# Zeudon/sound-event-localization-detection

Hardware: AMD Instinct MI355X
Metric: training clips/sec (4ch FOA 60s@24kHz) (higher is better)
Workload: dtype bf16; 1 GPU; crnn FOA 4-ch 60s clips, bs=32 windows (BASELINE configs[1]); parallelism=dp1

## Files before the change

### include/seld_hip.h

```cpp
#ifndef SELD_HIP_H_
#define SELD_HIP_H_

#include <stdint.h>

#ifdef __cplusplus
extern "C" {
#endif

int seld_init(int device);
int seld_shutdown(void);
int seld_version(void);
const char* seld_last_error(void);

int seld_set_mel_filterbank(const float* fb_host);

int seld_set_window(const float* window_host);

int seld_default_tables(float* window960, float* fb481x64, int* mel_b0_64, float* mel_wd_24x64,
                        float* mel_wu_24x64);

int64_t seld_num_frames(int64_t L);

int seld_logmel_f32(const float* pcm, int64_t N, int64_t C, int64_t L, float* out, int layout, void* stream);
int seld_logmel_i16(const int16_t* pcm, int64_t N, int64_t C, int64_t L, float* out, int layout, void* stream);
// ... 114 lines not shown
                         seld_guard_record* guard, void* stream);

int seld_multi_adam_guarded(const void* const* grad, const int32_t* grad_is_bf16, float* const* param,
                            float* const* exp_avg, float* const* exp_avg_sq, void* const* low_bf16, const int64_t* lengths,
                            int count, const float* lr, const float* step, float beta1, float beta2, float eps,
                            float weight_decay, float grad_scale, float* const* ema, float ema_decay,
                            const seld_guard_record* guard, void* stream);

int seld_multi_cast(const void* const* src, void* const* dst, const int64_t* lengths, int count, int bf16_to_fp32,
                    void* stream);

int seld_layernorm_supported(int64_t D);
int64_t seld_layernorm_workspace_floats(int64_t rows, int64_t D);
int seld_layernorm_forward(const void* x, int is_bf16, int64_t rows, int64_t D, const float* weight, const float* bias,
                           float eps, int relu, void* y, float* mean_rstd, void* stream);
int seld_layernorm_backward(const void* x, const void* dy, int is_bf16, int64_t rows, int64_t D, const float* weight,
                            const float* bias, const float* mean_rstd, int relu, void* dx, float* dweight,
                            float* dbias, float* workspace, void* stream);

int seld_stream_delay(int64_t nanoseconds, void* stream);

int64_t seld_smr_loss_workspace_bytes(int64_t frames, int64_t cells_per_frame);
int seld_smr_loss(const void* logits, int logits_is_bf16, const uint16_t* mask, const float* dense_labels,
                  int64_t frames, int rows, int cols, int num_classes, float w_class, float w_aiur, float w_cl,
                  float* loss_out4, void* grad, void* workspace, void* stream);


int seld_gru_fold_bias(const float* b_ih, const float* b_hh, int64_t H, void* gi_bias, int out_is_bf16, float* b_hn,
                       void* stream);

int seld_gru_prepare(const float* b_ih, const float* b_hh, const void* w_hh, int w_is_bf16, int64_t H, void* gi_bias,
                     int out_is_bf16, float* b_hn, void* w_hh_t_bf16, void* stream);

int seld_gru_bias_grads(const float* partial, int64_t tiles, int64_t H, float* db_ih, float* db_hh, void* stream);

int seld_sum_chunks(const void* partial, int in_is_bf16, int64_t chunks, int64_t count, void* out, int out_is_bf16,
                    void* stream);

int seld_sum_chunks_columns(const void* partial, int in_is_bf16, int64_t chunks, int64_t rows, int64_t C, int64_t F,
                            void* out, int out_is_bf16, void* stream);

int64_t seld_column_sums_blocks(int64_t rows, int64_t n_cols);
int seld_column_sums(const void* g, int in_is_bf16, int64_t rows, int64_t n_cols, float* partial, void* out, int out_is_bf16,
                     void* stream);

int seld_multi_sum_chunks(const void* const* partial, void* const* out, const int64_t* counts, const int32_t* chunks,
                          const int32_t* flags, int count, void* stream);
int seld_multi_column_sums_scratch(const int64_t* rows, const int64_t* n_cols, int count, int64_t* partial_floats);
int seld_multi_column_sums(const void* const* g, void* const* out, const int64_t* rows, const int64_t* n_cols,
                           const int32_t* flags, int count, float* partial, int64_t partial_floats, void* stream);

int seld_gru_dwhh_finish(const void* p_gi, const void* p_n, int in_is_bf16, int64_t chunks, int64_t H, void* dw_hh,
                         int out_is_bf16, void* stream);

int seld_conv_weight_flip_transpose(const void* w, int elem_bytes, int64_t O, int64_t I, void* wt, void* stream);

int seld_conv3x3_wgrad_supported(int64_t F, int64_t Cin, int64_t Cout);
int64_t seld_conv3x3_wgrad_workspace_floats(int64_t B, int64_t T, int64_t F, int64_t Cin, int64_t Cout);
int seld_conv3x3_wgrad(const void* x, const void* dy, int64_t B, int64_t T, int64_t F, int64_t Cin, int64_t Cout,
                       void* dw, int dw_is_bf16, float* workspace, void* stream);

int seld_conv3x3_dgrad_supported(int64_t F, int64_t Cin, int64_t Cout);
int seld_conv3x3_dgrad(const void* dy, const void* w, int64_t B, int64_t T, int64_t F, int64_t Cin, int64_t Cout,
                       void* dx, void* stream);

int seld_convfirst_supported(int64_t F, int64_t Cin, int64_t Cout);
int64_t seld_convfirst_workspace_floats(int backward);
int seld_convfirst_forward(const void* in, const void* w, int w_is_bf16, int64_t w_sco, int64_t w_sci, int64_t w_sr,
                           int64_t w_ss, int64_t B, int64_t T, int64_t F, const float* bn_weight, const float* bn_bias,
                           float* running_mean, float* running_var, float momentum, float eps, void* y,
                           float* mean_invstd, float* scale_shift, float* workspace, int phases, void* stream);
int seld_convfirst_backward(const void* in, const void* w, int w_is_bf16, int64_t w_sco, int64_t w_sci, int64_t w_sr,
                            int64_t w_ss, const void* dy, int64_t B, int64_t T, int64_t F, const float* mean_invstd,
                            const float* scale_shift, void* dw, int dw_is_bf16, int64_t dw_sco, int64_t dw_sci,
                            int64_t dw_sr, int64_t dw_ss, float* dgamma, float* dbeta, float* workspace, int phases,
                            void* stream);

int64_t seld_conv_tail_workspace_floats(int C);
int seld_conv_tail_forward(const void* x, const void* residual, int is_bf16, int64_t rows, int C, int pool,
                           const float* weight, const float* bias, float* running_mean, float* running_var,
                           float momentum, float eps, int training, void* y, float* mean_invstd, float* scale_shift,
                           float* workspace, void* stream);
int seld_conv_tail_backward(const void* x, const void* residual, const void* dy, int is_bf16, int64_t rows, int C,
                            int pool, const float* mean_invstd, const float* scale_shift, void* dx, void* dresidual,
                            float* dweight, float* dbias, float* workspace, void* stream);

int seld_dwconv1d(const void* x, int is_bf16, const float* weight, const float* bias, int64_t B, int64_t T, int D, int K,
                  int flip_taps, void* y, void* stream);
int64_t seld_dwconv1d_wgrad_rows(int64_t B, int64_t T);
int seld_dwconv1d_wgrad(const void* x, const void* dy, int is_bf16, int64_t B, int64_t T, int D, int K, float* partial,
                        void* stream);

int64_t seld_gru_tile_rows(void);
int seld_gru_forward(const void* gi, int is_bf16, const void* w_hh_bf16, const float* b_hn, int64_t B,
                     int64_t T, int64_t H, void* y, void* saved_tile, void* stream);

int seld_gru_backward(const void* dy_tile, const void* saved_tile, const void* y, int is_bf16,
                      const void* w_hh_t_bf16, int64_t tiles, int64_t T, int64_t H, void* dg_tile, float* dbias,
                      void* stream);

int seld_gru_backward_direct(const void* dy, const void* saved_tile, const void* y, int is_bf16,
                             const void* w_hh_t_bf16, int64_t B, int64_t T, int64_t H, void* dgi, void* dghn,
                             float* dbias, void* stream);

int seld_gru_to_tile(const void* src, int elem_bytes, int64_t B, int64_t T, int ns, void* dst, void* stream);
int seld_gru_from_pair_tile(const void* dg_tile, int elem_bytes, int64_t B, int64_t T, void* dgi, void* dghn,
// ... 64 lines not shown
```

### sound-event-localization-detection_amd/csrc/conv3x3_image.h

```cpp
#pragma once

#include <hip/hip_runtime.h>

namespace seld {
namespace conv3x3 {

typedef __attribute__((ext_vector_type(8))) __bf16 bf16x8;
typedef __attribute__((ext_vector_type(4))) short s16x4;
typedef __attribute__((ext_vector_type(8))) short s16x8;
typedef __attribute__((ext_vector_type(4))) float f32x4;
typedef __attribute__((address_space(3))) s16x4 lds_s16x4;

constexpr int kThreads = 256;
constexpr int kChannels = 64;
constexpr int kPitch = 80;

template <int F, int P>
struct Image {
  static_assert(F == 8 || F == 16 || F == 32, "frequency bins: 8, 16 or 32");
  static_assert(P % F == 0, "a chunk is whole time rows");
  static constexpr int TC = P / F;
  static constexpr int kRows = (TC + 2) * (F + 2);
  static constexpr int kLoads = (kRows * 8 + kThreads - 1) / kThreads;
};

template <int F>
__device__ __forceinline__ int image_row(int pos) {
  return (pos / F + 1) * (F + 2) + pos % F + 1;
}

template <int F>
__device__ __forceinline__ constexpr int tap_shift(int tap) {
  return (tap / 3 - 1) * (F + 2) + (tap % 3 - 1);
}

template <int F, int P>
__device__ __forceinline__ uint4 image_piece(const unsigned short* __restrict__ src, long clip_row, int t0, int T,
                                             int C, int c0, int piece) {
  const int r = piece >> 3, ch = piece & 7;
  const int tr = r / (F + 2), f = r - tr * (F + 2) - 1, t = t0 - 1 + tr;
  uint4 v = make_uint4(0u, 0u, 0u, 0u);
  if (r < Image<F, P>::kRows && t >= 0 && t < T && f >= 0 && f < F)
    v = *reinterpret_cast<const uint4*>(src + ((clip_row + t) * F + f) * C + c0 + ch * 8);
  return v;
}

__device__ __forceinline__ s16x4 tr_read(const unsigned short* base, int offset_shorts) {
  return __builtin_amdgcn_ds_read_tr16_b64_v4i16((lds_s16x4*)(base + offset_shorts));
}

__device__ __forceinline__ bf16x8 join(s16x4 lo, s16x4 hi) {
  const s16x8 v = __builtin_shufflevector(lo, hi, 0, 1, 2, 3, 4, 5, 6, 7);
  return __builtin_bit_cast(bf16x8, v);
}

}
}
```

### sound-event-localization-detection_amd/csrc/convwgrad.hip

```cpp
#include <hip/hip_bf16.h>

#include "conv3x3_image.h"
#include "seld_common.h"

namespace seld {

namespace {

using namespace conv3x3;

constexpr int kWgThreads = 512;
constexpr int kWgTile = 64;
constexpr int kWgKc = 128;
constexpr int kWgPitch = kPitch;
constexpr int kWgSumThreads = 256;
constexpr int kWgSumRows = 8;

template <int F>
struct WgradGeom {
  using Img = Image<F, kWgKc>;
  static constexpr int TC = Img::TC;
  static constexpr int XR = Img::kRows;
  static constexpr int kDyLoads = kWgKc * 8 / kWgThreads;
  static constexpr int kXLoads = (XR * 8 + kWgThreads - 1) / kWgThreads;
// ... 140 lines not shown
    }
  part[row][col] = s;
  __syncthreads();
  if (row != 0 || i >= count) return;
#pragma unroll
  for (int r = 1; r < kWgSumRows; ++r) {
    const float4 v = part[r][col];
    s.x += v.x; s.y += v.y; s.z += v.z; s.w += v.w;
  }
  if (kBf16) {
    const unsigned lo = static_cast<unsigned>(__bfloat16_as_ushort(__float2bfloat16(s.x))) |
                        (static_cast<unsigned>(__bfloat16_as_ushort(__float2bfloat16(s.y))) << 16);
    const unsigned hi = static_cast<unsigned>(__bfloat16_as_ushort(__float2bfloat16(s.z))) |
                        (static_cast<unsigned>(__bfloat16_as_ushort(__float2bfloat16(s.w))) << 16);
    *reinterpret_cast<uint2*>(static_cast<unsigned short*>(dw) + i) = make_uint2(lo, hi);
  } else {
    *reinterpret_cast<float4*>(static_cast<float*>(dw) + i) = s;
  }
}

struct WgradPlan {
  int chunks_per_clip = 0, chunks = 0, per_slab = 0, slabs = 0;
};

int time_rows_per_chunk(int64_t F) { return static_cast<int>(kWgKc / F); }

bool wgrad_supported(int64_t F, int64_t Cin, int64_t Cout) {
  return (F == 8 || F == 16 || F == 32) && Cin > 0 && Cout > 0 && Cin % kWgTile == 0 &&
         Cout % kWgTile == 0;
}

WgradPlan wgrad_plan(int64_t B, int64_t T, int64_t F, int64_t Cin, int64_t Cout, int num_cus) {
  WgradPlan pl;
  const int tc = time_rows_per_chunk(F);
  pl.chunks_per_clip = static_cast<int>((T + tc - 1) / tc);
  pl.chunks = static_cast<int>(B) * pl.chunks_per_clip;
  const long tiles = (Cin / kWgTile) * (Cout / kWgTile);
  const long want = ((num_cus > 0 ? num_cus : 256) + tiles - 1) / tiles;
  const long slabs = want < 1 ? 1 : (want > pl.chunks ? pl.chunks : want);
  pl.per_slab = static_cast<int>((pl.chunks + slabs - 1) / slabs);
  pl.slabs = (pl.chunks + pl.per_slab - 1) / pl.per_slab;
  return pl;
}

template <int F>
void launch_wgrad(const unsigned short* x, const unsigned short* dy, int T, int Cin, int Cout, const WgradPlan& pl,
                  float* ws, hipStream_t stream) {
  const dim3 grid(static_cast<unsigned>(Cin / kWgTile), static_cast<unsigned>(Cout / kWgTile),
                  static_cast<unsigned>(pl.slabs));
  hipLaunchKernelGGL(conv3x3_wgrad_kernel<F>, grid, dim3(kWgThreads), 0, stream, x, dy, T, Cin, Cout,
                     pl.chunks_per_clip, pl.chunks, pl.per_slab, ws);
}

}

}

extern "C" {

int seld_conv3x3_wgrad_supported(int64_t F, int64_t Cin, int64_t Cout) {
  return seld::wgrad_supported(F, Cin, Cout) ? 1 : 0;
}

int64_t seld_conv3x3_wgrad_workspace_floats(int64_t B, int64_t T, int64_t F, int64_t Cin, int64_t Cout) {
  using namespace seld;
  const DeviceState* st = current_state();
  if (!st || B <= 0 || T <= 0 || !wgrad_supported(F, Cin, Cout)) return 0;
  return static_cast<int64_t>(wgrad_plan(B, T, F, Cin, Cout, st->num_cus).slabs) * Cout * 9 * Cin;
}

int seld_conv3x3_wgrad(const void* x, const void* dy, int64_t B, int64_t T, int64_t F, int64_t Cin, int64_t Cout,
                       void* dw, int dw_is_bf16, float* workspace, void* stream_) {
  using namespace seld;
  const DeviceState* st = current_state();
  if (!st) return kErrNotInitialised;
  if (!x || !dy || !dw || !workspace || B <= 0 || T <= 0)
    return fail(kErrInvalidArgument, "seld_conv3x3_wgrad: bad argument");
  if (!wgrad_supported(F, Cin, Cout))
    return fail(kErrUnsupported, "seld_conv3x3_wgrad: F in {8, 16, 32} and channel counts % 64 == 0 required");
  if (((reinterpret_cast<uintptr_t>(x) | reinterpret_cast<uintptr_t>(dy) | reinterpret_cast<uintptr_t>(dw) |
        reinterpret_cast<uintptr_t>(workspace)) & 15) != 0)
    return fail(kErrInvalidArgument, "seld_conv3x3_wgrad: 16-byte aligned tensors required");
  const WgradPlan pl = wgrad_plan(B, T, F, Cin, Cout, st->num_cus);
  hipStream_t stream = static_cast<hipStream_t>(stream_);
  const unsigned short* xs = static_cast<const unsigned short*>(x);
  const unsigned short* ds = static_cast<const unsigned short*>(dy);
  const int t = static_cast<int>(T), ci = static_cast<int>(Cin), co = static_cast<int>(Cout);
  switch (F) {
    case 8: launch_wgrad<8>(xs, ds, t, ci, co, pl, workspace, stream); break;
    case 16: launch_wgrad<16>(xs, ds, t, ci, co, pl, workspace, stream); break;
    default: launch_wgrad<32>(xs, ds, t, ci, co, pl, workspace, stream); break;
  }
  SELD_HIP_TRY(hipGetLastError());
  const long count = static_cast<long>(Cout) * 9 * Cin;
  const long cols = kWgSumThreads / kWgSumRows;
  const dim3 grid(static_cast<unsigned>((count / 4 + cols - 1) / cols));
  if (dw_is_bf16)
    hipLaunchKernelGGL(conv3x3_wgrad_sum_kernel<true>, grid, dim3(kWgSumThreads), 0, stream, workspace, pl.slabs,
                       count, dw);
  else
    hipLaunchKernelGGL(conv3x3_wgrad_sum_kernel<false>, grid, dim3(kWgSumThreads), 0, stream, workspace, pl.slabs,
                       count, dw);
  SELD_HIP_TRY(hipGetLastError());
  return kOk;
}

}
```

### sound-event-localization-detection_amd/seld_gru.py

```python
import torch
import torch.nn.functional as F

import seld_native
import seld_overlap
from seld_linear import chunk_count, tall_chunks, tall_product

HIDDEN = 256
direct_backward = True


def applicable(module, x):
    low = torch.is_autocast_enabled() or x.dtype in (torch.bfloat16, torch.float16)
    if not low and not getattr(module, "allow_fp32", False):
        return False
    return (module.hidden_size == HIDDEN and module.bidirectional and module.batch_first and module.bias
            and x.dim() == 3 and x.dtype in (torch.float32, torch.bfloat16, torch.float16) and module.proj_size == 0)


class _BiGRULayer(torch.autograd.Function):
    @staticmethod
    def forward(ctx, x, w_ih, b_ih, w_hh, b_hh, overlap=False, feature_cf=None):
        ctx.overlap = overlap
        ctx.feature_cf = feature_cf
        if feature_cf is not None:
            c, f = feature_cf
            w_ih = w_ih.view(w_ih.shape[0], c, f).transpose(1, 2).reshape(w_ih.shape[0], f * c)
        low = torch.is_autocast_enabled() or x.dtype == torch.bfloat16
        cdt = torch.bfloat16 if low else torch.float32
        with torch.autocast(device_type="cuda", enabled=False):
            xc = x.to(cdt)
            need = x.requires_grad or w_ih.requires_grad or w_hh.requires_grad
            w_hh_t = None
            if b_ih.dtype == torch.float32 and b_hh.dtype == torch.float32 and b_ih.is_contiguous() and b_hh.is_contiguous():
                if (direct_backward and need and w_hh.is_contiguous()
                        and w_hh.dtype in (torch.float32, torch.bfloat16)):
                    gi_bias, b_hn, w_hh_t = seld_native.gru_prepare(b_ih, b_hh.reshape(-1), w_hh, cdt)
                else:
                    gi_bias, b_hn = seld_native.gru_fold_bias(b_ih, b_hh.reshape(-1), cdt)
            else:
                fold = b_hh.clone()
                fold[:, 2 * HIDDEN:] = 0
                gi_bias, b_hn = (b_ih + fold.reshape(-1)).to(cdt), b_hh[:, 2 * HIDDEN:]
            gi = F.linear(xc, w_ih.to(cdt), gi_bias)
            b, t, _ = gi.shape
            y, saved = seld_native.gru_forward(gi.view(b, t, 2, 3 * HIDDEN), w_hh, b_hn, need)
        ctx.save_for_backward(xc, w_ih, w_hh, y, saved if saved is not None else torch.empty(0),
                              w_hh_t if w_hh_t is not None else torch.empty(0))
        ctx.cdt = cdt
        ctx.dtypes = (w_ih.dtype, b_ih.dtype, w_hh.dtype, b_hh.dtype)
        return y

    @staticmethod
    def backward(ctx, dy):
        xc, w_ih, w_hh, y, saved, w_hh_t = ctx.saved_tensors
        cdt = ctx.cdt
        b, t, _ = y.shape
        h = HIDDEN
        n = b * t
        with torch.autocast(device_type="cuda", enabled=False):
            dyc = dy.to(y.dtype)
            seld_overlap.launch_pending(dy.device)
            dgi, dghn, dbias = seld_native.gru_backward(dyc, saved, y, w_hh, raw_bias=True,
                                                        w_hh_t=w_hh_t if w_hh_t.numel() else None, direct=direct_backward)
            dgi2 = dgi.view(n, 6 * h)
            x2 = xc.reshape(n, -1)
            t_wih, t_bih, t_whh, t_bhh = ctx.dtypes

            dw_ih = torch.empty((6 * h, x2.shape[1]), dtype=t_wih, device=dy.device)
            dw_hh = torch.empty((2, 3 * h, h), dtype=t_whh, device=dy.device)
            db_ih = torch.empty(6 * h, dtype=t_bih, device=dy.device)
            db_hh = torch.empty(6 * h, dtype=t_bhh, device=dy.device)

            def weight_grads():
                fp32 = [db if db.dtype == torch.float32 else torch.empty(6 * h, dtype=torch.float32, device=dy.device)
                        for db in (db_ih, db_hh)]
                seld_native.gru_bias_grads(dbias, out=fp32)
                for db, full in zip((db_ih, db_hh), fp32):
                    if db is not full:
                        db.copy_(full)
                tall_product(dgi2, x2, out=dw_ih, columns_cf=ctx.feature_cf)
                hp = seld_native.gru_previous_state(y).view(n, 2 * h)
                chunks = chunk_count(n, 6 * h, 2 * h)
                p_gi = tall_chunks(dgi2, hp, chunks)
                p_n = tall_chunks(dghn.view(n, 2 * h), hp, chunks)
                seld_native.gru_dwhh_finish(p_gi, p_n, dw_hh)

            dx = (dgi2 @ w_ih.to(cdt)).view_as(xc)
            if ctx.overlap:
                seld_overlap.submit(dy.device, [dgi, dghn, y, xc, dbias, dw_ih, dw_hh, db_ih, db_hh], weight_grads)
            elif seld_overlap.conv_wgrad_side and seld_overlap.enabled and dy.is_cuda:
                seld_overlap.launch_now(dy.device, [dgi, dghn, y, xc, dbias, dw_ih, dw_hh, db_ih, db_hh], weight_grads,
                                        last_of_stage=True, outputs=[dw_ih, dw_hh, db_ih, db_hh])
            else:
                weight_grads()
        return dx.to(dy.dtype) if dx.dtype != dy.dtype and not torch.is_autocast_enabled() else dx, \
            dw_ih.view_as(dw_ih), db_ih.view_as(db_ih), dw_hh.view_as(dw_hh), db_hh.view(2, 3 * h), None, None


from seld_pack import adjacent as _adjacent, join as _join, pack as _pack


def pack_parameters(module):
    with torch.no_grad():
        for layer in range(module.num_layers):
            for kind in ("weight_ih", "bias_ih", "weight_hh", "bias_hh"):
                _pack((getattr(module, f"{kind}_l{layer}"), getattr(module, f"{kind}_l{layer}_reverse")))


def bigru_forward(module, x, feature_cf=None, overlap=False, need_hn=True):
    overlap = overlap and seld_overlap.active(x)
    params = []
    for layer in range(module.num_layers):
        p = lambda name: getattr(module, f"{name}_l{layer}")
        pr = lambda name: getattr(module, f"{name}_l{layer}_reverse")
        group = (_join(p("weight_ih"), pr("weight_ih")), _join(p("bias_ih"), pr("bias_ih")),
                 _join(p("weight_hh"), pr("weight_hh")), _join(p("bias_hh"), pr("bias_hh")))
        params.append(seld_overlap.defer(*group) if overlap and layer > 0 else group)
    out = x
    finals = []
    for layer in range(module.num_layers):
        w_ih, b_ih, w_hh, b_hh = params[layer]
        out = _BiGRULayer.apply(out, w_ih, b_ih, w_hh.view(2, 3 * HIDDEN, HIDDEN), b_hh.view(2, 3 * HIDDEN),
                                overlap and layer > 0, feature_cf if layer == 0 else None)
        if need_hn:
            finals += [out[:, -1, :HIDDEN], out[:, 0, HIDDEN:]]
        if module.training and module.dropout > 0 and layer + 1 < module.num_layers:
            out = F.dropout(out, p=module.dropout, training=True)
    return out, (torch.stack(finals, dim=0) if need_hn else None)
```

### sound-event-localization-detection_amd/seld_native.py

```python
from __future__ import annotations

import ctypes
import os
import threading
from pathlib import Path

import torch

from seld_augment import PARAM_INTS as AUGMENT_PARAM_INTS, PATTERNS as AUGMENT_PATTERNS, check_channel_order

_HERE = Path(__file__).resolve().parent
LIB_PATH = Path(os.environ["SELD_HIP_LIB"]).resolve() if os.environ.get("SELD_HIP_LIB") else _HERE / "libseld_hip.so"

N_FFT = 960
HOP = 480
N_BINS = 481
N_MELS = 64

_lock = threading.Lock()
_lib = None
_initialised_devices = set()

_i64 = ctypes.c_int64
_int = ctypes.c_int
# ... 22 lines not shown
    for name in ("seld_stft_f32", "seld_stft_i16"):
        getattr(lib, name).argtypes = [_ptr, _i64, _i64, _i64, _ptr, _ptr]
    lib.seld_foa_intensity.argtypes = [_ptr, _i64, _i64, _ptr, _i64, _i64, _i64, _i64, _ptr]
    for fn in (lib.seld_logmel_iv_f32, lib.seld_logmel_iv_i16):
        fn.argtypes = [_ptr, _i64, _i64, _ptr, _i64, _i64, _i64, _i64, _ptr]
    for fn in (lib.seld_logmel_spectrum_f32, lib.seld_logmel_spectrum_i16):
        fn.argtypes = [_ptr, _i64, _i64, _i64, _ptr, _i64, _i64, _i64, _i64, _ptr, _ptr]
        fn.restype = ctypes.c_int
    for fn in (lib.seld_logmel_phasors_f32, lib.seld_logmel_phasors_i16):
        fn.argtypes = [_ptr, _i64, _i64, _i64, _ptr, _i64, _i64, _i64, _i64, _ptr, _ptr]
    lib.seld_phasor_pitch.restype = ctypes.c_int64
    lib.seld_gcc_phat_q15.argtypes = [_ptr, _i64, _i64, _i64, _ptr, _i64, _i64, _i64, _i64, _ptr]
    lib.seld_gcc_table_host.argtypes = [_ptr]
    lib.seld_gcc_phat.argtypes = [_ptr, _i64, _i64, _i64, _ptr, _i64, _i64, _i64, _i64, _ptr]
    lib.seld_labels_rasterise.argtypes = [_ptr, _i64, _i64, _int, _int, _ptr, _ptr]
    lib.seld_labels_expand.argtypes = [_ptr, _i64, _int, _ptr, _ptr]
    lib.seld_labels_rasterise_box.argtypes = [_ptr, _ptr, _i64, _i64, _int, _int, ctypes.c_double, ctypes.c_double, _ptr,
                                              _ptr]
    lib.seld_window_gather.argtypes = [_ptr, _i64, _i64, _ptr, _i64, _i64, _ptr, _ptr]
    lib.seld_window_gather_augment.argtypes = [_ptr, _i64, _int, _int, _ptr, _ptr, _i64, _i64, _ptr, ctypes.c_float, _ptr, _ptr]
    lib.seld_window_permute_mask.argtypes = [_ptr, _i64, _int, _int, _ptr, _ptr, _i64, _i64, _ptr, _ptr]
    lib.seld_foa_rotation_terms.argtypes = [_ptr, _i64, _i64, _int, _int, _ptr, _i64, _i64, _i64, _i64, _ptr]
    lib.seld_window_gather_rotate.argtypes = [_ptr, _ptr, _i64, _int, _int, _int, _int, _int, _int, _ptr, _ptr, _i64, _i64, _ptr,
                                              ctypes.c_float, _ptr, _ptr]
    lib.seld_window_permute_mask_rotate.argtypes = [_ptr, _i64, _int, _int, _ptr, _ptr, _i64, _i64, _ptr, _ptr]
    lib.seld_feature_moments_workspace.restype = _i64
    lib.seld_feature_moments_workspace.argtypes = [_i64, _int]
    lib.seld_feature_moments.argtypes = [_ptr, _i64, _int, _ptr, _ptr, _i64, _ptr]
    lib.seld_window_gather_affine.argtypes = [_ptr, _i64, _int, _ptr, _i64, _i64, _ptr, _ptr, _ptr, _ptr]
    lib.seld_window_gather_augment_affine.argtypes = [_ptr, _i64, _int, _int, _ptr, _ptr, _i64, _i64, _ptr, ctypes.c_float,
                                                      _ptr, _ptr, _ptr, _ptr]
    lib.seld_window_gather_rotate_affine.argtypes = [_ptr, _ptr, _i64, _int, _int, _int, _int, _int, _int, _ptr, _ptr, _i64,
                                                     _i64, _ptr, ctypes.c_float, _ptr, _ptr, _ptr, _ptr]
    lib.seld_softmax_mse_workspace_bytes.restype = _i64
    lib.seld_softmax_mse_workspace_bytes.argtypes = []
    lib.seld_softmax_mse.argtypes = [_ptr, _int, _ptr, _ptr, _i64, _int, ctypes.c_float, _ptr, _ptr, _ptr, _ptr]
    lib.seld_softmax_ce_workspace_bytes.restype = _i64
    lib.seld_softmax_ce_workspace_bytes.argtypes = []
    lib.seld_softmax_ce.argtypes = [_ptr, _int, _ptr, _ptr, _i64, _int, _ptr, ctypes.c_float, ctypes.c_float, _ptr, _ptr,
                                    _ptr, _ptr]
    lib.seld_scale_by_device_scalar.argtypes = [_ptr, _int, _i64, _ptr, _ptr]
    lib.seld_smr_loss_workspace_bytes.restype = _i64
    lib.seld_smr_loss_workspace_bytes.argtypes = [_i64, _i64]
    lib.seld_smr_loss.argtypes = [_ptr, _int, _ptr, _ptr, _i64, _int, _int, _int, ctypes.c_float, ctypes.c_float,
                                  ctypes.c_float, _ptr, _ptr, _ptr, _ptr]
    lib.seld_multi_cast.argtypes = [_ptr, _ptr, _ptr, _int, _int, _ptr]
    lib.seld_stream_delay.argtypes = [_i64, _ptr]
    lib.seld_gru_fold_bias.argtypes = [_ptr, _ptr, _i64, _ptr, _int, _ptr, _ptr]
    lib.seld_gru_prepare.argtypes = [_ptr, _ptr, _ptr, _int, _i64, _ptr, _int, _ptr, _ptr, _ptr]
    lib.seld_gru_bias_grads.argtypes = [_ptr, _i64, _i64, _ptr, _ptr, _ptr]
    lib.seld_sum_chunks.argtypes = [_ptr, _int, _i64, _i64, _ptr, _int, _ptr]
    lib.seld_sum_chunks_columns.argtypes = [_ptr, _int, _i64, _i64, _i64, _i64, _ptr, _int, _ptr]
    lib.seld_gru_dwhh_finish.argtypes = [_ptr, _ptr, _int, _i64, _i64, _ptr, _int, _ptr]
    lib.seld_column_sums.argtypes = [_ptr, _int, _i64, _i64, _ptr, _ptr, _int, _ptr]
    _pp, _pi64, _pi32 = ctypes.POINTER(ctypes.c_void_p), ctypes.POINTER(ctypes.c_int64), ctypes.POINTER(ctypes.c_int32)
    _f = ctypes.c_float
    lib.seld_multi_adam.argtypes = [_pp, _pi32, _pp, _pp, _pp, _pp, _pi64, _int, _ptr, _ptr, _f, _f, _f, _f, _f, _ptr]
    lib.seld_multi_grad_norm_scratch.argtypes = [_pi64, _int, _pi64]
    lib.seld_multi_grad_norm.argtypes = [_pp, _pi32, _pi64, _int, _f, _f, _int, _ptr, _i64, _ptr, _ptr]
    lib.seld_multi_adam_guarded.argtypes = [_pp, _pi32, _pp, _pp, _pp, _pp, _pi64, _int, _ptr, _ptr, _f, _f, _f, _f, _f, _pp, _f,
                                            _ptr, _ptr]
    lib.seld_multi_sum_chunks.argtypes = [_pp, _pp, _pi64, _pi32, _pi32, _int, _ptr]
    lib.seld_multi_column_sums_scratch.argtypes = [_pi64, _pi64, _int, _pi64]
    lib.seld_multi_column_sums.argtypes = [_pp, _pp, _pi64, _pi64, _pi32, _int, _ptr, _i64, _ptr]
    lib.seld_column_sums_blocks.argtypes = [_i64, _i64]
    lib.seld_column_sums_blocks.restype = ctypes.c_int64
    lib.seld_conv_weight_flip_transpose.argtypes = [_ptr, _int, _i64, _i64, _ptr, _ptr]
    lib.seld_conv3x3_wgrad_supported.argtypes = [_i64, _i64, _i64]
    lib.seld_conv3x3_wgrad_workspace_floats.restype = _i64
    lib.seld_conv3x3_wgrad_workspace_floats.argtypes = [_i64, _i64, _i64, _i64, _i64]
    lib.seld_conv3x3_wgrad.argtypes = [_ptr, _ptr, _i64, _i64, _i64, _i64, _i64, _ptr, _int, _ptr, _ptr]
    lib.seld_conv3x3_dgrad_supported.argtypes = [_i64, _i64, _i64]
    lib.seld_conv3x3_dgrad.argtypes = [_ptr, _ptr, _i64, _i64, _i64, _i64, _i64, _ptr, _ptr]
    lib.seld_convfirst_supported.argtypes = [_i64, _i64, _i64]
    lib.seld_convfirst_workspace_floats.restype = _i64
    lib.seld_convfirst_workspace_floats.argtypes = [_int]
    lib.seld_convfirst_forward.argtypes = [_ptr, _ptr, _int, _i64, _i64, _i64, _i64, _i64, _i64, _i64, _ptr, _ptr, _ptr, _ptr,
                                           ctypes.c_float, ctypes.c_float, _ptr, _ptr, _ptr, _ptr, _int, _ptr]
    lib.seld_convfirst_backward.argtypes = [_ptr, _ptr, _int, _i64, _i64, _i64, _i64, _ptr, _i64, _i64, _i64, _ptr, _ptr,
                                            _ptr, _int, _i64, _i64, _i64, _i64, _ptr, _ptr, _ptr, _int, _ptr]
    lib.seld_layernorm_supported.argtypes = [_i64]
    lib.seld_layernorm_workspace_floats.restype = _i64
    lib.seld_layernorm_workspace_floats.argtypes = [_i64, _i64]
    lib.seld_layernorm_forward.argtypes = [_ptr, _int, _i64, _i64, _ptr, _ptr, ctypes.c_float, _int, _ptr, _ptr, _ptr]
    lib.seld_layernorm_backward.argtypes = [_ptr, _ptr, _int, _i64, _i64, _ptr, _ptr, _ptr, _int, _ptr, _ptr, _ptr,
                                            _ptr, _ptr]
    lib.seld_conv_tail_workspace_floats.restype = _i64
    lib.seld_conv_tail_workspace_floats.argtypes = [_int]
    lib.seld_conv_tail_forward.argtypes = [_ptr, _ptr, _int, _i64, _int, _int, _ptr, _ptr, _ptr, _ptr, ctypes.c_float,
                                           ctypes.c_float, _int, _ptr, _ptr, _ptr, _ptr, _ptr]
    lib.seld_conv_tail_backward.argtypes = [_ptr, _ptr, _ptr, _int, _i64, _int, _int, _ptr, _ptr, _ptr, _ptr, _ptr, _ptr,
                                            _ptr, _ptr]
    lib.seld_dwconv1d.argtypes = [_ptr, _int, _ptr, _ptr, _i64, _i64, _int, _int, _int, _ptr, _ptr]
    lib.seld_dwconv1d_wgrad.argtypes = [_ptr, _ptr, _int, _i64, _i64, _int, _int, _ptr, _ptr]
    lib.seld_dwconv1d_wgrad_rows.argtypes = [_i64, _i64]
    lib.seld_dwconv1d_wgrad_rows.restype = ctypes.c_int64
    lib.seld_gru_to_tile.argtypes = [_ptr, _int, _i64, _i64, _int, _ptr, _ptr]
    lib.seld_gru_from_pair_tile.argtypes = [_ptr, _int, _i64, _i64, _ptr, _ptr, _ptr]
    lib.seld_gru_previous_state.argtypes = [_ptr, _int, _i64, _i64, _ptr, _ptr]
    lib.seld_gru_tile_rows.restype = _i64
    lib.seld_gru_tile_rows.argtypes = []
    lib.seld_gru_forward.argtypes = [_ptr, _int, _ptr, _ptr, _i64, _i64, _i64, _ptr, _ptr, _ptr]
    lib.seld_gru_backward.argtypes = [_ptr, _ptr, _ptr, _int, _ptr, _i64, _i64, _i64, _ptr, _ptr, _ptr]
    lib.seld_gru_backward_direct.argtypes = [_ptr, _ptr, _ptr, _int, _ptr, _i64, _i64, _i64, _ptr, _ptr, _ptr, _ptr]
    lib.seld_grid_decode.argtypes = [_ptr, _int, _i64, _i64, _i64, _i64, _ptr, _ptr, _i64, _i64, ctypes.c_float, _int,
                                     _ptr, _ptr, _ptr, _ptr, _ptr]
# ... 1197 lines not shown
    with _device_guard(ensure_init(device)):
        check(load_library().seld_multi_sum_chunks(src, dst, counts, chunks, flags, n, _stream_ptr(device)),
              "seld_multi_sum_chunks")


_column_scratch = {}
_retired_scratch = []


def multi_column_sums(pairs) -> None:
    pairs = list(pairs)
    if not pairs:
        return
    for g, out in pairs:
        if not column_sums_supported(g, out):
            raise SeldNativeError("multi_column_sums: g [rows, N] contiguous bf16 / fp32 with N % 8 == 0, out [N] contiguous")
    lib = load_library()
    n = len(pairs)
    src = (ctypes.c_void_p * n)(*[g.data_ptr() for g, _ in pairs])
    dst = (ctypes.c_void_p * n)(*[o.data_ptr() for _, o in pairs])
    rows = (ctypes.c_int64 * n)(*[g.shape[0] for g, _ in pairs])
    cols = (ctypes.c_int64 * n)(*[g.shape[1] for g, _ in pairs])
    flags = (ctypes.c_int32 * n)(*[_is_bf16(g) | (_is_bf16(o) << 1) for g, o in pairs])
    need_f = ctypes.c_int64(0)
    check(lib.seld_multi_column_sums_scratch(rows, cols, n, ctypes.byref(need_f)), "seld_multi_column_sums_scratch")
    device = pairs[0][0].device
    index = ensure_init(device)
    scratch = _column_scratch.get(index)
    if scratch is None or scratch.numel() < need_f.value:
        if torch.cuda.is_current_stream_capturing():
            raise SeldNativeError("multi_column_sums: the scratch must be sized by an eager call before a graph capture")
        if scratch is not None:
            _retired_scratch.append(scratch)
        scratch = torch.empty(max(need_f.value, 1 << 20), dtype=torch.float32, device=device)
        _column_scratch[index] = scratch
    with _device_guard(index):
        check(lib.seld_multi_column_sums(src, dst, rows, cols, flags, n, _p(scratch), scratch.numel(), _stream_ptr(device)),
              "seld_multi_column_sums")


def gru_dwhh_finish(p_gi: torch.Tensor, p_n: torch.Tensor, out: torch.Tensor) -> torch.Tensor:
    chunks = p_gi.shape[0]
    h = out.shape[2]
    if not (p_gi.is_contiguous() and p_n.is_contiguous() and out.is_contiguous() and p_gi.dtype == p_n.dtype
            and tuple(p_gi.shape) == (chunks, 6 * h, 2 * h) and tuple(p_n.shape) == (chunks, 2 * h, 2 * h)
            and tuple(out.shape) == (2, 3 * h, h)):
        raise SeldNativeError("gru_dwhh_finish: shapes must be [chunks, 6H, 2H], [chunks, 2H, 2H] -> [2, 3H, H]")
    with _device_guard(ensure_init(out.device)):
        check(load_library().seld_gru_dwhh_finish(_p(p_gi), _p(p_n), _is_bf16(p_gi), chunks, h, _p(out), _is_bf16(out),
                                                  _stream_ptr(out.device)), "seld_gru_dwhh_finish")
    return out


def conv_weight_flip_transpose(w: torch.Tensor) -> torch.Tensor:
    o, i, kh, kw = w.shape
    if not (w.is_cuda and kh == 3 and kw == 3 and w.dtype in (torch.float32, torch.bfloat16)
            and w.is_contiguous(memory_format=torch.channels_last)):
        raise SeldNativeError("conv_weight_flip_transpose: 3x3 weights in channels-last memory expected")
    wt = torch.empty((i, o, 3, 3), dtype=w.dtype, device=w.device, memory_format=torch.channels_last)
    with _device_guard(ensure_init(w.device)):
        check(load_library().seld_conv_weight_flip_transpose(_p(w), w.element_size(), o, i, _p(wt),
                                                             _stream_ptr(w.device)), "seld_conv_weight_flip_transpose")
    return wt


def conv3x3_wgrad_applicable(x: torch.Tensor, dy: torch.Tensor, w: torch.Tensor) -> bool:
    if not (x.is_cuda and x.dim() == 4 and dy.dim() == 4 and w.dim() == 4 and x.dtype == torch.bfloat16
            and dy.dtype == torch.bfloat16 and tuple(w.shape[2:]) == (3, 3)):
        return False
    b, cin, t, f = x.shape
    if tuple(dy.shape) != (b, w.shape[0], t, f) or w.shape[1] != cin:
        return False
    if not (x.is_contiguous(memory_format=torch.channels_last) and dy.is_contiguous(memory_format=torch.channels_last)
            and w.is_contiguous(memory_format=torch.channels_last)):
        return False
    return bool(load_library().seld_conv3x3_wgrad_supported(f, cin, w.shape[0]))


def conv3x3_wgrad(x: torch.Tensor, dy: torch.Tensor, dw: torch.Tensor) -> torch.Tensor:
    if not conv3x3_wgrad_applicable(x, dy, dw) or dw.dtype not in (torch.float32, torch.bfloat16):
        raise SeldNativeError("conv3x3_wgrad: unsupported shapes, dtypes or layouts")
    b, cin, t, f = x.shape
    cout = dy.shape[1]
    with _device_guard(ensure_init(x.device)):
        lib = load_library()
        ws = torch.empty(int(lib.seld_conv3x3_wgrad_workspace_floats(b, t, f, cin, cout)), dtype=torch.float32,
                         device=x.device)
        check(lib.seld_conv3x3_wgrad(_p(x), _p(dy), b, t, f, cin, cout, _p(dw), _is_bf16(dw), _p(ws),
                                     _stream_ptr(x.device)), "seld_conv3x3_wgrad")
    return dw


def conv3x3_dgrad_applicable(dy: torch.Tensor, w: torch.Tensor) -> bool:
    if not (dy.is_cuda and dy.dim() == 4 and w.dim() == 4 and dy.dtype == torch.bfloat16 and w.dtype == torch.bfloat16
            and tuple(w.shape[2:]) == (3, 3) and dy.shape[1] == w.shape[0]):
        return False
    if not (dy.is_contiguous(memory_format=torch.channels_last) and w.is_contiguous(memory_format=torch.channels_last)):
        return False
    return bool(load_library().seld_conv3x3_dgrad_supported(dy.shape[3], w.shape[1], w.shape[0]))


def conv3x3_dgrad(dy: torch.Tensor, w: torch.Tensor, out: "torch.Tensor | None" = None) -> torch.Tensor:
    if not conv3x3_dgrad_applicable(dy, w):
        raise SeldNativeError("conv3x3_dgrad: unsupported shapes, dtypes or layouts")
    b, cout, t, f = dy.shape
    cin = w.shape[1]
# ... 128 lines not shown
```

Baseline: 172.8 clips/s.

## Fuse GRU recurrent weight gradient into one MFMA kernel with slab reduction

Adds a dedicated HIP kernel that computes the GRU hidden-to-hidden weight gradient directly from dgi, dghn and the output sequence. It reads the time-shifted previous state on the fly, so no gathered previous-state tensor is built. It accumulates per-slab partials with bf16 MFMA and double-buffered LDS, then reduces them with the shared slab-sum kernel, which is factored out of the conv wgrad path. This replaces the old gather, tall-chunk products and finish steps, cutting kernel launches and intermediate traffic. The cost is a fixed H=256 specialisation and a workspace allocation on every call.

Result: no change. 172.6 clips/s, median of 2 (-0.1%).

```diff
diff --git a/include/seld_hip.h b/include/seld_hip.h
--- a/include/seld_hip.h
+++ b/include/seld_hip.h
@@ -190,6 +190,10 @@
 
 int seld_gru_dwhh_finish(const void* p_gi, const void* p_n, int in_is_bf16, int64_t chunks, int64_t H, void* dw_hh,
                          int out_is_bf16, void* stream);
+
+int64_t seld_gru_dwhh_workspace_floats(int64_t B, int64_t T, int64_t H);
+int seld_gru_dwhh(const void* dgi, const void* dghn, const void* y, int in_is_bf16, int64_t B, int64_t T, int64_t H,
+                  void* dw_hh, int out_is_bf16, float* workspace, void* stream);
 
 int seld_conv_weight_flip_transpose(const void* w, int elem_bytes, int64_t O, int64_t I, void* wt, void* stream);
 
diff --git a/sound-event-localization-detection_amd/csrc/conv3x3_image.h b/sound-event-localization-detection_amd/csrc/conv3x3_image.h
--- a/sound-event-localization-detection_amd/csrc/conv3x3_image.h
+++ b/sound-event-localization-detection_amd/csrc/conv3x3_image.h
@@ -54,5 +54,7 @@
   return __builtin_bit_cast(bf16x8, v);
 }
 
+hipError_t slab_sum(const float* ws, int slabs, long count, void* out, bool out_is_bf16, hipStream_t stream);
+
 }
 }
diff --git a/sound-event-localization-detection_amd/csrc/convwgrad.hip b/sound-event-localization-detection_amd/csrc/convwgrad.hip
--- a/sound-event-localization-detection_amd/csrc/convwgrad.hip
+++ b/sound-event-localization-detection_amd/csrc/convwgrad.hip
@@ -216,6 +216,16 @@
                      pl.chunks_per_clip, pl.chunks, pl.per_slab, ws);
 }
 
+}
+
+hipError_t conv3x3::slab_sum(const float* ws, int slabs, long count, void* out, bool out_is_bf16, hipStream_t stream) {
+  const long cols = kWgSumThreads / kWgSumRows;
+  const dim3 grid(static_cast<unsigned>((count / 4 + cols - 1) / cols));
+  if (out_is_bf16)
+    hipLaunchKernelGGL(conv3x3_wgrad_sum_kernel<true>, grid, dim3(kWgSumThreads), 0, stream, ws, slabs, count, out);
+  else
+    hipLaunchKernelGGL(conv3x3_wgrad_sum_kernel<false>, grid, dim3(kWgSumThreads), 0, stream, ws, slabs, count, out);
+  return hipGetLastError();
 }
 
 }
@@ -256,16 +266,7 @@
     default: launch_wgrad<32>(xs, ds, t, ci, co, pl, workspace, stream); break;
   }
   SELD_HIP_TRY(hipGetLastError());
-  const long count = static_cast<long>(Cout) * 9 * Cin;
-  const long cols = kWgSumThreads / kWgSumRows;
-  const dim3 grid(static_cast<unsigned>((count / 4 + cols - 1) / cols));
-  if (dw_is_bf16)
-    hipLaunchKernelGGL(conv3x3_wgrad_sum_kernel<true>, grid, dim3(kWgSumThreads), 0, stream, workspace, pl.slabs,
-                       count, dw);
-  else
-    hipLaunchKernelGGL(conv3x3_wgrad_sum_kernel<false>, grid, dim3(kWgSumThreads), 0, stream, workspace, pl.slabs,
-                       count, dw);
-  SELD_HIP_TRY(hipGetLastError());
+  SELD_HIP_TRY(slab_sum(workspace, pl.slabs, static_cast<long>(Cout) * 9 * Cin, dw, dw_is_bf16 != 0, stream));
   return kOk;
 }
 
diff --git a/sound-event-localization-detection_amd/csrc/grudwhh.hip b/sound-event-localization-detection_amd/csrc/grudwhh.hip
--- /dev/null
+++ b/sound-event-localization-detection_amd/csrc/grudwhh.hip
@@ -0,0 +1,184 @@
+#include <hip/hip_bf16.h>
+
+#include "conv3x3_image.h"
+#include "seld_common.h"
+
+namespace seld {
+
+namespace {
+
+using namespace conv3x3;
+
+constexpr int kDwThreads = 512;
+constexpr int kDwH = 256;
+constexpr int kDwKc = 64;
+constexpr int kDwM = kDwH;
+constexpr int kDwN = 128;
+constexpr int kDwSubM = kDwM / kChannels, kDwSubN = kDwN / kChannels;
+constexpr int kDwSubShorts = kDwKc * kPitch;
+constexpr int kDwImageShorts = (kDwSubM + kDwSubN) * kDwSubShorts;
+constexpr int kDwLdsShorts = 2 * kDwImageShorts;
+constexpr int kDwGroup = 3 * (kDwH / kDwN);
+constexpr long kDwCount = 2L * 3 * kDwH * kDwH;
+static_assert(kDwThreads == kDwKc * 8, "one 16-byte piece of every sub-image row per thread");
+static_assert(kDwLdsShorts * 2 > 80 * 1024 && kDwLdsShorts * 2 <= 124 * 1024, "LDS footprint outside its bracket");
+
+constexpr int kDwLaunchBound = 2 * kDwThreads;
+static_assert(kDwLaunchBound == 1024, "the register budget is 512 / (bound waves per SIMD)");
+
+__global__ __launch_bounds__(kDwLaunchBound) void gru_dwhh_kernel(
+    const unsigned short* __restrict__ dgi, const unsigned short* __restrict__ dghn, const unsigned short* __restrict__ y,
+    int T, int chunks_per_clip, int chunks, int per_slab, int groups, float* __restrict__ ws) {
+  __shared__ __attribute__((aligned(16))) unsigned short lds[kDwLdsShorts];
+
+  const int lane = threadIdx.x & 63, wave = threadIdx.x >> 6;
+  const int wm = wave >> 1, wn = wave & 1;
+  const int xcd = blockIdx.x & 7, j = blockIdx.x >> 3;
+  const int group = (j / kDwGroup) * 8 + xcd, member = j % kDwGroup;
+  if (group >= groups) return;
+  const int nb = member & 1, gate = member >> 1, d = group & 1, slab = group >> 1;
+  const int c_begin = slab * per_slab;
+  const int c_end = min(c_begin + per_slab, chunks);
+  const unsigned short* const gsrc = gate < 2 ? dgi + (d * 3 + gate) * kDwH : dghn + d * kDwH;
+  const int gstride = gate < 2 ? 6 * kDwH : 2 * kDwH;
+  const unsigned short* const ysrc = y + d * kDwH + nb * kDwN;
+  const int shift = d == 0 ? -1 : 1;
+
+  f32x4 acc[4][4];
+#pragma unroll
+  for (int m = 0; m < 4; ++m)
+#pragma unroll
+    for (int n = 0; n < 4; ++n) acc[m][n] = f32x4{0.0f, 0.0f, 0.0f, 0.0f};
+
+  uint4 rg[kDwSubM], ry[kDwSubN];
+  bool in_g, in_y;
+  auto load = [&](int c) {
+    int tid = threadIdx.x;
+    asm volatile("" : "+v"(tid));
+    const int b = c / chunks_per_clip, t0 = (c - b * chunks_per_clip) * kDwKc;
+    const long row0 = static_cast<long>(b) * T + t0;
+    const int pos = tid >> 3, ch8 = (tid & 7) * 8, ty = t0 + pos + shift;
+    in_g = t0 + pos < T;
+    in_y = in_g && ty >= 0 && ty < T;
+    const unsigned short* const g0 = gsrc + row0 * gstride + (in_g ? pos * gstride : 0) + ch8;
+    const unsigned short* const y0 = ysrc + row0 * (2 * kDwH) + (in_y ? (pos + shift) * (2 * kDwH) : 0) + ch8;
+#pragma unroll
+    for (int i = 0; i < kDwSubM; ++i) rg[i] = *reinterpret_cast<const uint4*>(g0 + i * kChannels);
+#pragma unroll
+    for (int i = 0; i < kDwSubN; ++i) ry[i] = *reinterpret_cast<const uint4*>(y0 + i * kChannels);
+  };
+  auto store = [&](unsigned short* image) {
+    int tid = threadIdx.x;
+    asm volatile("" : "+v"(tid));
+    auto piece_or_zero = [](uint4 v, bool inside) {
+      return make_uint4(inside ? v.x : 0u, inside ? v.y : 0u, inside ? v.z : 0u, inside ? v.w : 0u);
+    };
+    unsigned short* const at = image + (tid >> 3) * kPitch + (tid & 7) * 8;
+#pragma unroll
+    for (int i = 0; i < kDwSubM; ++i) *reinterpret_cast<uint4*>(at + i * kDwSubShorts) = piece_or_zero(rg[i], in_g);
+#pragma unroll
+    for (int i = 0; i < kDwSubN; ++i)
+      *reinterpret_cast<uint4*>(at + (kDwSubM + i) * kDwSubShorts) = piece_or_zero(ry[i], in_y);
+  };
+
+  if (c_begin < c_end) {
+    load(c_begin);
+    store(lds);
+  }
+  for (int c = c_begin; c < c_end; ++c) {
+    __syncthreads();
+    const bool more = c + 1 < c_end;
+    if (more) load(c + 1);
+    int lt = threadIdx.x;
+    asm volatile("" : "+v"(lt));
+    const int g = (lt >> 4) & 3, q = (lt >> 2) & 3, p = lt & 3, wv = lt >> 6;
+    const int lpos = 4 * g + q;
+    const unsigned short* const image = lds + ((c - c_begin) & 1) * kDwImageShorts;
+    const unsigned short* const pa = image + (wv >> 1) * kDwSubShorts + lpos * kPitch + 4 * p;
+    const unsigned short* const pb = image + (kDwSubM + (wv & 1)) * kDwSubShorts + lpos * kPitch + 4 * p;
+#pragma unroll 1
+    for (int ks = 0; ks < kDwKc / 32; ++ks) {
+      const unsigned short* const ka = pa + ks * 32 * kPitch;
+      const unsigned short* const kb = pb + ks * 32 * kPitch;
+      bf16x8 a[4];
+#pragma unroll
+      for (int m = 0; m < 4; ++m) a[m] = join(tr_read(ka, m * 16), tr_read(ka, 16 * kPitch + m * 16));
+#pragma unroll
+      for (int n = 0; n < 4; ++n) {
+        const bf16x8 bfr = join(tr_read(kb, n * 16), tr_read(kb, 16 * kPitch + n * 16));
+#pragma unroll
+        for (int m = 0; m < 4; ++m)
+          acc[m][n] = __builtin_amdgcn_mfma_f32_16x16x32_bf16(a[m], bfr, acc[m][n], 0, 0, 0);
+      }
+    }
+    if (more) store(lds + ((c + 1 - c_begin) & 1) * kDwImageShorts);
+  }
+
+  float* const slot = ws + slab * kDwCount + static_cast<long>(d * 3 + gate) * kDwH * kDwH;
+#pragma unroll
+  for (int m = 0; m < 4; ++m)
+#pragma unroll
+    for (int j = 0; j < 4; ++j) {
+      const int u = wm * 64 + m * 16 + 4 * (lane >> 4) + j;
+#pragma unroll
+      for (int n = 0; n < 4; ++n) slot[u * kDwH + nb * kDwN + wn * 64 + n * 16 + (lane & 15)] = acc[m][n][j];
+    }
+}
+
+struct DwhhPlan {
+  int chunks_per_clip = 0, chunks = 0, per_slab = 0, slabs = 0;
+};
+
+DwhhPlan dwhh_plan(int64_t B, int64_t T, int num_cus) {
+  DwhhPlan pl;
+  pl.chunks_per_clip = static_cast<int>((T + kDwKc - 1) / kDwKc);
+  pl.chunks = static_cast<int>(B) * pl.chunks_per_clip;
+  const long want = (num_cus > 0 ? num_cus : 256) / 32;
+  const long slabs = want < 1 ? 1 : (want > pl.chunks ? pl.chunks : want);
+  pl.per_slab = static_cast<int>((pl.chunks + slabs - 1) / slabs);
+  pl.slabs = (pl.chunks + pl.per_slab - 1) / pl.per_slab;
+  return pl;
+}
+
+bool dwhh_shape_ok(int64_t B, int64_t T, int64_t H) {
+  return H == kDwH && B > 0 && T > 0 && B * ((T + kDwKc - 1) / kDwKc) <= (1 << 24);
+}
+
+}
+
+}
+
+extern "C" {
+
+int64_t seld_gru_dwhh_workspace_floats(int64_t B, int64_t T, int64_t H) {
+  using namespace seld;
+  const DeviceState* st = current_state();
+  if (!st || !dwhh_shape_ok(B, T, H)) return 0;
+  return dwhh_plan(B, T, st->num_cus).slabs * kDwCount;
+}
+
+int seld_gru_dwhh(const void* dgi, const void* dghn, const void* y, int in_is_bf16, int64_t B, int64_t T, int64_t H,
+                  void* dw_hh, int out_is_bf16, float* workspace, void* stream_) {
+  using namespace seld;
+  const DeviceState* st = current_state();
+  if (!st) return kErrNotInitialised;
+  if (!dgi || !dghn || !y || !dw_hh || !workspace || B <= 0 || T <= 0)
+    return fail(kErrInvalidArgument, "seld_gru_dwhh: bad argument");
+  if (!in_is_bf16 || !dwhh_shape_ok(B, T, H))
+    return fail(kErrUnsupported, "seld_gru_dwhh: bf16 dgi / dghn / y and H = 256 required");
+  if (((reinterpret_cast<uintptr_t>(dgi) | reinterpret_cast<uintptr_t>(dghn) | reinterpret_cast<uintptr_t>(y) |
+        reinterpret_cast<uintptr_t>(dw_hh) | reinterpret_cast<uintptr_t>(workspace)) & 15) != 0)
+    return fail(kErrInvalidArgument, "seld_gru_dwhh: 16-byte aligned tensors required");
+  const DwhhPlan pl = dwhh_plan(B, T, st->num_cus);
+  hipStream_t stream = static_cast<hipStream_t>(stream_);
+  const int groups = 2 * pl.slabs;
+  const dim3 grid(static_cast<unsigned>((groups + 7) / 8 * 8 * kDwGroup));
+  hipLaunchKernelGGL(gru_dwhh_kernel, grid, dim3(kDwThreads), 0, stream, static_cast<const unsigned short*>(dgi),
+                     static_cast<const unsigned short*>(dghn), static_cast<const unsigned short*>(y),
+                     static_cast<int>(T), pl.chunks_per_clip, pl.chunks, pl.per_slab, groups, workspace);
+  SELD_HIP_TRY(hipGetLastError());
+  SELD_HIP_TRY(slab_sum(workspace, pl.slabs, kDwCount, dw_hh, out_is_bf16 != 0, stream));
+  return kOk;
+}
+
+}
diff --git a/sound-event-localization-detection_amd/seld_gru.py b/sound-event-localization-detection_amd/seld_gru.py
--- a/sound-event-localization-detection_amd/seld_gru.py
+++ b/sound-event-localization-detection_amd/seld_gru.py
@@ -1,3 +1,5 @@
+import os
+
 import torch
 import torch.nn.functional as F
 
@@ -7,6 +9,8 @@
 
 HIDDEN = 256
 direct_backward = True
+fused_dwhh = os.environ.get("SELD_FUSED_DWHH", "1") != "0"
+dwhh_first = os.environ.get("SELD_DWHH_FIRST", "1") != "0"
 
 
 def applicable(module, x):
@@ -78,7 +82,14 @@
                 for db, full in zip((db_ih, db_hh), fp32):
                     if db is not full:
                         db.copy_(full)
+                fused = fused_dwhh and seld_native.gru_dwhh_applicable(dgi, dghn, y, dw_hh)
+                if fused and dwhh_first:
+                    seld_native.gru_dwhh(dgi, dghn, y, dw_hh)
                 tall_product(dgi2, x2, out=dw_ih, columns_cf=ctx.feature_cf)
+                if fused and not dwhh_first:
+                    seld_native.gru_dwhh(dgi, dghn, y, dw_hh)
+                if fused:
+                    return
                 hp = seld_native.gru_previous_state(y).view(n, 2 * h)
                 chunks = chunk_count(n, 6 * h, 2 * h)
                 p_gi = tall_chunks(dgi2, hp, chunks)
diff --git a/sound-event-localization-detection_amd/seld_native.py b/sound-event-localization-detection_amd/seld_native.py
--- a/sound-event-localization-detection_amd/seld_native.py
+++ b/sound-event-localization-detection_amd/seld_native.py
@@ -98,6 +98,9 @@
     lib.seld_sum_chunks.argtypes = [_ptr, _int, _i64, _i64, _ptr, _int, _ptr]
     lib.seld_sum_chunks_columns.argtypes = [_ptr, _int, _i64, _i64, _i64, _i64, _ptr, _int, _ptr]
     lib.seld_gru_dwhh_finish.argtypes = [_ptr, _ptr, _int, _i64, _i64, _ptr, _int, _ptr]
+    lib.seld_gru_dwhh_workspace_floats.restype = _i64
+    lib.seld_gru_dwhh_workspace_floats.argtypes = [_i64, _i64, _i64]
+    lib.seld_gru_dwhh.argtypes = [_ptr, _ptr, _ptr, _int, _i64, _i64, _i64, _ptr, _int, _ptr, _ptr]
     lib.seld_column_sums.argtypes = [_ptr, _int, _i64, _i64, _ptr, _ptr, _int, _ptr]
     _pp, _pi64, _pi32 = ctypes.POINTER(ctypes.c_void_p), ctypes.POINTER(ctypes.c_int64), ctypes.POINTER(ctypes.c_int32)
     _f = ctypes.c_float
@@ -1401,6 +1404,29 @@
     return out
 
 
+def gru_dwhh_applicable(dgi: torch.Tensor, dghn: torch.Tensor, y: torch.Tensor, out: torch.Tensor) -> bool:
+    if not (dgi.is_cuda and dgi.dim() == 5 and dgi.dtype == dghn.dtype == y.dtype == torch.bfloat16
+            and dgi.device == dghn.device == y.device == out.device and out.dtype in (torch.float32, torch.bfloat16)):
+        return False
+    b, t = dgi.shape[:2]
+    return (b > 0 and t > 0 and tuple(dgi.shape) == (b, t, 2, 3, GRU_H) and tuple(dghn.shape) == (b, t, 2, GRU_H)
+            and tuple(y.shape) == (b, t, 2 * GRU_H) and tuple(out.shape) == (2, 3 * GRU_H, GRU_H)
+            and dgi.is_contiguous() and dghn.is_contiguous() and y.is_contiguous() and out.is_contiguous())
+
+
+def gru_dwhh(dgi: torch.Tensor, dghn: torch.Tensor, y: torch.Tensor, out: torch.Tensor) -> torch.Tensor:
+    if not gru_dwhh_applicable(dgi, dghn, y, out):
+        raise SeldNativeError("gru_dwhh: contiguous bf16 dgi [B, T, 2, 3, 256], dghn [B, T, 2, 256], y [B, T, 512] and "
+                              "out [2, 768, 256] (fp32 / bf16) on one GPU required")
+    b, t = dgi.shape[:2]
+    with _device_guard(ensure_init(dgi.device)):
+        lib = load_library()
+        ws = torch.empty(int(lib.seld_gru_dwhh_workspace_floats(b, t, GRU_H)), dtype=torch.float32, device=dgi.device)
+        check(lib.seld_gru_dwhh(_p(dgi), _p(dghn), _p(y), 1, b, t, GRU_H, _p(out), _is_bf16(out), _p(ws),
+                                _stream_ptr(dgi.device)), "seld_gru_dwhh")
+    return out
+
+
 def conv_weight_flip_transpose(w: torch.Tensor) -> torch.Tensor:
     o, i, kh, kw = w.shape
     if not (w.is_cuda and kh == 3 and kw == 3 and w.dtype in (torch.float32, torch.bfloat16)
```
